# usnistgov/alignn

Measured on AMD Instinct MI355X. Metric: graphs/sec (train fwd+bwd), batch=64 JARVIS-DFT crystals, 4+4 ALIGNN layers, higher is better.
Workload: dtype f32 (projections: split-product MFMA - 3 fp16-slice or 6 bf16-slice products, fp32 accumulate, fp32-grade error)

## Files before the change

alignn_amd/csrc/model.hip:

```cpp
#include <chrono>
#include <cstdio>
#include <cstdlib>
#include <vector>

#include "../../include/alignn_hip.h"
#include "common.h"

namespace {

constexpr int kEvents = 512;
constexpr int kAmaxSlots = 1024;

struct EventPool {
    hipEvent_t ev[kEvents];
    int next = 0;
    bool ok = false;
};
EventPool g_pool[kMaxDevices];

__global__ void fill_kernel(float* __restrict__ p, int64_t n, float v) {
    const int64_t i = (int64_t)blockIdx.x * blockDim.x + threadIdx.x;
    if (i < n) p[i] = v;
}
__global__ void bump_kernel(int64_t* const* __restrict__ ptrs, int n) {
    const int i = blockIdx.x * blockDim.x + threadIdx.x;
    if (i < n) ptrs[i][0] += 1;
}
__global__ __launch_bounds__(256) void transpose_kernel(const float* __restrict__ in, int64_t ld, int rows, int cols,
                                                        float* __restrict__ out) {
    __shared__ float tile[32][33];
    const int tx = threadIdx.x & 31, ty = threadIdx.x >> 5;
    const int r0 = blockIdx.y * 32, c0 = blockIdx.x * 32;
    for (int j = ty; j < 32; j += 8)
        if (r0 + j < rows && c0 + tx < cols) tile[j][tx] = in[(int64_t)(r0 + j) * ld + c0 + tx];
    __syncthreads();
    for (int j = ty; j < 32; j += 8)
        if (c0 + j < cols && r0 + tx < rows) out[(int64_t)(c0 + j) * rows + r0 + tx] = tile[tx][j];
}

struct Act {
    float* p = nullptr;
    float* amax = nullptr;
    float* xn = nullptr;
    float* stat = nullptr;
    float* red = nullptr;
    bool on_T = false;
};
struct Grad {
    float* p = nullptr;
    bool on_T = false;
    bool pre_red = false;
};

struct MlpTape {
    const alignn_mlp_params* p = nullptr;
    Act x, y;
    float *pre = nullptr, *stat = nullptr;
    int64_t rows = 0;
    bool lane = false;
};
struct ConvTape {
    const alignn_conv_params* p = nullptr;
    const alignn_graph_csr* g = nullptr;
    Act x, y, x_out, y_out;
    float *P = nullptr, *M = nullptr, *xpre = nullptr, *s0 = nullptr, *hh = nullptr, *n_stat = nullptr, *e_stat = nullptr;
    bool lane = false, need_y = true;
};
struct Tape {
    float *bl = nullptr, *rbf_e = nullptr, *rbf_a = nullptr, *pool = nullptr;
    float *hcos_buf = nullptr, *pred = nullptr, *seed = nullptr, *g_r = nullptr;
    const float* hcos = nullptr;
    bool angle_fused = false, angle_lane = false;
    float *a_stat1 = nullptr, *a_stat2 = nullptr, *a_scal = nullptr;
    MlpTape atom, e1, e2, a1, a2;
    std::vector<ConvTape> convs;
};

std::vector<std::pair<size_t, size_t>> g_dbg_allocs;
bool dbg_allocs_on() {
    static int on = -1;
    if (on < 0) on = getenv("ALIGNN_AMD_DEBUG_ALLOCS") ? 1 : 0;
    return on == 1;
}

struct Ctx {
    const alignn_model_desc* d;
    const alignn_model_batch* b;
    char* base;
    size_t off = 0, cap = 0;
    bool launch = false;
    bool unsupported = false;
    int unsupported_line = 0;
    int rc = 0;
    hipStream_t main = nullptr, T = nullptr, side = nullptr, aux = nullptr;
    float* amax_arena = nullptr;
    int amax_next = 0;
    EventPool* pool = nullptr;

    float* alloc(size_t floats) {
        const size_t bytes = al256(floats * sizeof(float));
        float* p = reinterpret_cast<float*>(base + off);
        if (launch && dbg_allocs_on()) g_dbg_allocs.emplace_back(off, bytes);
        off += bytes;
        if (launch && off > cap && rc == 0) rc = (int)hipErrorInvalidValue;
        return p;
    }
    size_t sbase[4] = {0, 0, 0, 0}, scur[4] = {0, 0, 0, 0}, speak[4] = {0, 0, 0, 0};
    int which(hipStream_t st) const { return st == main ? 0 : st == T ? 1 : st == side ? 2 : 3; }
    void tmp_reset(hipStream_t st) { scur[which(st)] = 0; }
    float* tmp(hipStream_t st, size_t floats) {
// ... 7 lines not shown
    }
    float* new_amax() {
        if (amax_next >= kAmaxSlots) {
            if (rc == 0) rc = (int)hipErrorInvalidValue;
            return amax_arena;
        }
        return amax_arena + amax_next++;
    }
    float* new_amax2() {
        if (amax_next + 2 > kAmaxSlots) {
            if (rc == 0) rc = (int)hipErrorInvalidValue;
            return amax_arena;
        }
        amax_next += 2;
        return amax_arena + amax_next - 2;
    }
    bool track(int64_t rows) const { return rows >= d->amax_min_rows; }
    const alignn_ff_desc* ff = nullptr;
    bool param_grads = true;
    bool geom = false;
    float *g_rbf_e = nullptr, *g_rbf_a = nullptr;
    bool g_rbf_a_on_T = false;
    ptrdiff_t toff = 0;
    float* sink = nullptr;
    int64_t sink_floats = 0;
    ptrdiff_t sink_toff = 0;
    float* twin(float* dW) const { return dW + ((sink != nullptr && dW >= sink && dW < sink + sink_floats) ? sink_toff : toff); }
    int n_sync = 0, n_launch = 0;
    double t_sync = 0.0;
    bool timing = false;
    void sync(hipStream_t waiter, hipStream_t src) {
        if (!launch || rc != 0 || waiter == src) return;
        const auto t0 = timing ? std::chrono::steady_clock::now() : std::chrono::steady_clock::time_point();
        hipEvent_t e = pool->ev[pool->next];
        pool->next = (pool->next + 1) % kEvents;
        rc = (int)hipEventRecord(e, src);
        if (rc == 0) rc = (int)hipStreamWaitEvent(waiter, e, 0);
        ++n_sync;
        if (timing) t_sync += std::chrono::duration<double>(std::chrono::steady_clock::now() - t0).count();
    }
};

#define UNSUP()                         \
    do {                                \
        c.unsupported = true;           \
        if (!c.unsupported_line) c.unsupported_line = __LINE__; \
    } while (0)

#define L(call)                                                                                        \
    do {                                                                                               \
        if (c.launch && c.rc == 0) {                                                                   \
            c.rc = (call);                                                                             \
            ++c.n_launch;                                                                              \
            if (c.rc != 0 && getenv("ALIGNN_AMD_DEBUG")) fprintf(stderr, "model.hip:%d rc %d: %s\n", __LINE__, c.rc, #call); \
        }                                                                                              \
    } while (0)

inline bool x6_shape_ok(const Ctx& c, int64_t M, int64_t lda, int N, int K) {
    const int64_t tiles = ((M + 63) / 64) * ((N + 255) / 256);
    return tiles >= c.d->x6_min_tiles && (lda % 4) == 0 && alignn_gemm_nt_x6_supported(M, N, K) != 0;
}

void fill(Ctx& c, float* p, int64_t n, float v, hipStream_t st) {
    if (!c.launch || c.rc != 0 || n <= 0) return;
    hipLaunchKernelGGL(fill_kernel, dim3((unsigned)((n + 255) / 256)), dim3(256), 0, st, p, n, v);
    c.rc = (int)hipGetLastError();
}

void project(Ctx& c, const float* a, int64_t lda, const float* a_amax, const float* w, int64_t ldw, const void* img,
             const float* w_amax, const float* bias, float* out, int64_t ldo, int64_t M, int N, int K, hipStream_t st) {
    if (x6_shape_ok(c, M, lda, N, K)) {
        if (a_amax == nullptr || img == nullptr) {
// ... 7 lines not shown
}

void bn_finalize_folded(Ctx& c, float* partial, int slabs, int64_t rows, int F, const float* gamma, const float* beta,
                        float* rm, float* rv, float* stat, hipStream_t st) {
    if (slabs > kFoldAbove) {
        float* fold = c.alloc((size_t)alignn_slab_fold_slabs() * 2 * F);
        L(alignn_slab_fold(partial, slabs, 2 * F, fold, st));
        partial = fold;
        slabs = alignn_slab_fold_slabs();
    }
    L(alignn_bn_finalize(partial, slabs, rows, F, gamma, beta, c.d->eps, c.d->momentum, rm, rv, stat, st));
}

void bn_bwd_finalize_folded(Ctx& c, float* partial, int slabs, int F, float* red, hipStream_t st) {
    if (slabs > kFoldAbove) {
        float* fold = c.alloc((size_t)alignn_slab_fold_slabs() * 2 * F);
        L(alignn_slab_fold(partial, slabs, 2 * F, fold, st));
        partial = fold;
        slabs = alignn_slab_fold_slabs();
    }
    L(alignn_bn_bwd_finalize(partial, slabs, F, red, st));
}



Act mlp_fwd(Ctx& c, MlpTape& t, const alignn_mlp_params& p, const Act& x, int64_t rows) {
    const bool ln = c.d->norm == 1;
    const int F = p.out, K = p.in;
    t.p = &p;
    t.x = x;
    t.rows = rows;
    t.lane = c.T != c.main && rows >= c.d->lane_min_rows;
    hipStream_t st = t.lane ? c.T : c.main;
    if (t.lane != x.on_T) c.sync(st, x.on_T ? c.T : c.main);
    t.pre = c.alloc((size_t)rows * F);
    t.stat = c.alloc(ln ? (size_t)rows * 2 : (size_t)4 * F);
    const bool fused_stats = !ln && x.amax != nullptr && x6_shape_ok(c, rows, K, F, K);
    if (fused_stats) {
        if (p.img == nullptr) {
            UNSUP();
            return Act{};
        }
        const int tiles = alignn_gemm_nt_x6_row_tiles(rows, F, K);
        float* partial = c.alloc((size_t)(tiles + 1) * 2 * F);
        L(alignn_gemm_nt_f16x3_stats(x.p, K, x.amax, p.img, p.w_amax, p.b, t.pre, F, rows, F, K, partial, st));
        bn_finalize_folded(c, partial, tiles, rows, F, p.gamma, p.beta, p.rm, p.rv, t.stat, st);
    } else {
        project(c, x.p, K, x.amax, p.W, K, p.img, p.w_amax, p.b, t.pre, F, rows, F, K, st);
        if (!ln) {
            const int slabs = alignn_col_stats_slabs(rows);
            float* partial = c.alloc((size_t)slabs * (3 * F + 1));
            L(alignn_col_stats_welford(t.pre, F, rows, F, partial, st));
            L(alignn_bn_finalize_welford(partial, slabs, rows, F, p.gamma, p.beta, c.d->eps, c.d->momentum, p.rm, p.rv, t.stat, st));
        }
    }
    Act y;
    y.p = c.alloc((size_t)rows * F);
    y.amax = c.track(rows) ? c.new_amax() : nullptr;
    if (ln)
        L(alignn_ln_silu_fwd(t.pre, F, nullptr, 0, p.gamma, p.beta, c.d->eps, y.p, F, t.stat, rows, F, y.amax, st));
    else {
        L(alignn_bn_silu_fwd(t.pre, F, nullptr, 0, t.stat, y.p, F, rows, F, y.amax, st));
        y.xn = t.pre;
        y.stat = t.stat;
        y.red = p.red;
    }
    y.on_T = t.lane;
    t.y = y;
    return y;
}

void conv_fwd(Ctx& c, ConvTape& t, const alignn_conv_params& p, const alignn_graph_csr& g, const Act& x, const Act& y,
              bool need_y) {
    const bool ln = c.d->norm == 1;
    const int H = c.d->H, Kin = H;
    const int64_t n = g.n, m = g.m;
    t.p = &p;
    t.g = &g;
    t.x = x;
    t.y = y;
    t.need_y = need_y;
    t.lane = c.T != c.main && m >= c.d->lane_min_rows;
    hipStream_t main = c.main, T = t.lane ? c.T : c.main;
    if (x.on_T) c.sync(main, c.T);
    if (!t.lane && y.on_T) c.sync(main, c.T);
    t.P = c.alloc((size_t)n * 4 * H);
    project(c, x.p, Kin, x.amax, p.wcat, Kin, p.wcat_img, p.wcat_amax, p.bcat, t.P, 4 * H, n, 4 * H, Kin, main);
    t.xpre = c.alloc((size_t)n * H);
    t.s0 = c.alloc((size_t)n * H);
    t.hh = c.alloc((size_t)n * H);
    t.M = c.alloc((size_t)m * H);
    const int n_slabs = alignn_egc_slabs(n);
    float *n_part = nullptr, *e_part = nullptr;
    if (ln)
        t.n_stat = c.alloc((size_t)n * 2);
    else {
        n_part = c.alloc((size_t)n_slabs * (3 * H + 1));
        t.n_stat = c.alloc((size_t)8 * H);
        t.e_stat = t.n_stat + 4 * H;
    }
    const bool x6 = x6_shape_ok(c, m, Kin, H, Kin);
    const bool pre_added = y.amax != nullptr && x6;
    if (!pre_added && x6) UNSUP();
    if (t.lane) c.sync(T, main);
    Act yo;
    if (need_y) {
        yo.p = c.alloc((size_t)m * H);
        yo.amax = c.track(m) ? c.new_amax() : nullptr;
        if (ln) t.e_stat = c.alloc((size_t)m * 2);
        yo.on_T = t.lane;
    }
    bool y_normed = false;
    if (pre_added) {
        if (p.weg_img == nullptr) {
            UNSUP();
            return;
        }
        const int tiles = alignn_gemm_nt_x6_row_tiles(m, H, Kin);
        if (!ln) e_part = c.alloc((size_t)(tiles + 1) * 2 * H);
        if (c.d->bd_segment_table && g.seg_node != nullptr && g.seg_rank != nullptr) {
            float* bd2 = c.alloc((size_t)n * H);
            L(alignn_gather_rows_ld(t.P + H, 4 * H, g.seg_node, bd2, H, n, H, T));
            L(alignn_gemm_nt_f16x3_gather2(y.p, Kin, y.amax, p.weg_img, p.weg_amax, p.b_eg, t.M, H, m, H, Kin, t.P, 4 * H, g.src,
                                           bd2, H, g.seg_rank, e_part, T));
        } else
            L(alignn_gemm_nt_f16x3_gather(y.p, Kin, y.amax, p.weg_img, p.weg_amax, p.b_eg, t.M, H, m, H, Kin, t.P, 4 * H, g.src,
                                          g.dst, e_part, T));
        if (!ln) bn_finalize_folded(c, e_part, tiles, m, H, p.e_gamma, p.e_beta, p.e_rm, p.e_rv, t.e_stat, T);
        y_normed = need_y && (!ln || alignn_egc_ln_fused_supported(H, m));
        if (!y_normed)
            L(alignn_egc_gate_fwd_pre(t.P, t.M, g.seg_ptr, g.seg_node, g.src, n, m, H, t.xpre, t.s0, t.hh, nullptr, n_part, T));
        else if (ln)
            L(alignn_egc_gate_fwd_pre_ln(t.P, t.M, g.seg_ptr, g.seg_node, g.src, n, m, H, t.xpre, t.s0, t.hh, p.e_gamma, p.e_beta, c.d->eps,
                                         y.p, yo.p, t.e_stat, yo.amax, T));
        else
            L(alignn_egc_gate_fwd_pre_norm(t.P, t.M, g.seg_ptr, g.seg_node, g.src, n, m, H, t.xpre, t.s0, t.hh, n_part, t.e_stat,
                                           y.p, yo.p, yo.amax, T));
    } else {
        L(alignn_gemm_nt(y.p, Kin, p.w_eg, Kin, p.b_eg, nullptr, 0, t.M, H, m, H, Kin, T));
        if (!ln) e_part = c.alloc((size_t)n_slabs * (3 * H + 1));
        L(alignn_egc_gate_fwd(t.P, t.M, g.seg_ptr, g.seg_node, g.src, n, m, H, t.xpre, t.s0, t.hh, e_part, n_part, T));
    }
    if (t.lane) c.sync(main, T);
// ... 55 lines not shown
    fill(c, c.amax_arena, kAmaxSlots, 0.0f, c.main);
    const bool angle_first = c.ff == nullptr && d.norm == 0 && d.angle_fused != 0 && Tn > 0 && c.T != c.main && Tn >= d.lane_min_rows &&
                             alignn_angle_embed_supported(d.angle_bins, d.angle1.out, d.angle2.out) != 0;
    if (angle_first) c.sync(c.T, c.main);
    const bool prep_aside = angle_first && c.aux != c.main && d.n_weights > 0 && c.ff == nullptr &&
                            !x6_shape_ok(c, N, d.atom.in, d.atom.out, d.atom.in) &&
                            !x6_shape_ok(c, E, d.edge1.in, d.edge1.out, d.edge1.in);
    hipStream_t prep_st = prep_aside ? c.aux : c.main;
    if (prep_aside) c.sync(c.aux, c.main);
    if (d.n_weights > 0) L(alignn_prepare_weights(d.weight_descs, d.n_weights, d.weight_amax, prep_st));
    if (d.n_bump > 0 && c.launch && c.rc == 0) {
        hipLaunchKernelGGL(bump_kernel, dim3((d.n_bump + 63) / 64), dim3(64), 0, c.main, (int64_t* const*)d.bump_ptrs, d.n_bump);
        c.rc = (int)hipGetLastError();
    }
    tp.hcos = b.h;
    if (c.ff != nullptr && c.ff->lg_on_fly) {
        tp.hcos_buf = c.alloc((size_t)Tn);
        L(alignn_bond_cosine_fwd(b.r, b.lg.src, b.lg.dst, tp.hcos_buf, Tn, c.main));
        tp.hcos = tp.hcos_buf;
    }
    if (!angle_first) c.sync(c.T, c.main);
    Act z;
    tp.angle_fused = d.norm == 0 && d.angle_fused != 0 && Tn > 0 &&
                     alignn_angle_embed_supported(d.angle_bins, d.angle1.out, d.angle2.out) != 0;
    if (tp.angle_fused) {
        tp.angle_lane = c.T != c.main && Tn >= d.lane_min_rows;
        hipStream_t st = tp.angle_lane ? c.T : c.main;
        tp.a_stat1 = c.alloc((size_t)4 * d.angle1.out);
        tp.a_stat2 = c.alloc((size_t)4 * d.angle2.out);
        tp.a_scal = c.alloc((size_t)alignn_angle_embed_scal_floats());
        alignn_angle_args a = angle_args(c, tp);
        z.p = c.alloc((size_t)Tn * H);
        z.amax = c.track(Tn) ? c.new_amax() : nullptr;
        z.on_T = tp.angle_lane;
        a.z = z.p;
        a.z_amax = z.amax;
        a.workspace_bytes = alignn_angle_embed_workspace(Tn, d.angle_bins, 0);
        a.workspace = c.alloc(a.workspace_bytes / sizeof(float));
        L(alignn_angle_embed_fwd(&a, st));
    } else {
        tp.rbf_a = c.alloc((size_t)Tn * d.angle_bins);
        L(alignn_rbf_fwd(tp.hcos, d.angle_centers, d.angle_gamma, tp.rbf_a, Tn, d.angle_bins, c.main));
        Act za;
        za.p = tp.rbf_a;
        z = mlp_fwd(c, tp.a2, d.angle2, mlp_fwd(c, tp.a1, d.angle1, za, Tn), Tn);
    }
    Act xa;
    xa.p = const_cast<float*>(b.atom_features);
    Act x = mlp_fwd(c, tp.atom, d.atom, xa, N);
    tp.bl = c.alloc((size_t)E);
    L(alignn_norm3_fwd(b.r, tp.bl, E, c.main));
    tp.rbf_e = c.alloc((size_t)E * d.edge_bins);
    L(alignn_rbf_fwd(tp.bl, d.edge_centers, d.edge_gamma, tp.rbf_e, E, d.edge_bins, c.main));
    Act ye;
    ye.p = tp.rbf_e;
    Act y1 = mlp_fwd(c, tp.e1, d.edge1, ye, E);
    if (prep_aside) c.sync(c.main, c.aux);
    Act y = mlp_fwd(c, tp.e2, d.edge2, y1, E);
    if (c.unsupported) return;
    tp.convs.assign(conv_count(d), ConvTape{});
    int k = 0;
    for (int i = 0; i < d.alignn_layers; ++i) {
        ConvTape& tg = tp.convs[k];
        conv_fwd(c, tg, d.convs[k], b.g, x, y, true);
        ++k;
        ConvTape& tl = tp.convs[k];
        conv_fwd(c, tl, d.convs[k], b.lg, tg.y_out, z, i + 1 < d.alignn_layers);
        ++k;
        x = tg.x_out;
        y = tl.x_out;
        z = tl.y_out;
        if (c.unsupported) return;
    }
    for (int i = 0; i < d.gcn_layers; ++i) {
        ConvTape& tg = tp.convs[k];
        conv_fwd(c, tg, d.convs[k], b.g, x, y, i + 1 < d.gcn_layers);
        ++k;
        x = tg.x_out;
        y = tg.y_out;
        if (c.unsupported) return;
    }
    if (x.on_T) c.sync(c.main, c.T);
    tp.pool = c.alloc((size_t)b.B * H);
    L(alignn_segment_mean_fwd(x.p, b.graph_ptr, tp.pool, b.B, H, c.main));
    L(alignn_gemm_nt(tp.pool, H, d.fc_W, H, d.fc_b, nullptr, 0, out, d.out_features, b.B, d.out_features, H, c.main));
    c.sync(c.main, c.T);
}


void transpose(Ctx& c, const float* w, int64_t ld, int rows, int cols, float* out, hipStream_t st) {
    if (!c.launch || c.rc != 0) return;
    hipLaunchKernelGGL(transpose_kernel, dim3((cols + 31) / 32, (rows + 31) / 32), dim3(256), 0, st, w, ld, rows, cols, out);
    c.rc = (int)hipGetLastError();
}

void dgrad(Ctx& c, const float* g, int64_t ldg, const float* g_amax, const float* w, int Nred, int Kout, const void* img_t,
           const float* w_amax, const float* addend, int64_t ldadd, float* out, int64_t M, hipStream_t st, const Act* src,
           bool* pre_red) {
    if (pre_red) *pre_red = false;
    const bool x6 = x6_shape_ok(c, M, ldg, Kout, Nred);
    if (x6) {
        if (g_amax == nullptr || img_t == nullptr) {
            UNSUP();
            return;
        }
        if (src != nullptr && src->xn != nullptr) {
            const int tiles = alignn_gemm_nt_x6_row_tiles(M, Kout, Nred);
            float* part = c.alloc((size_t)(tiles + 1) * 2 * Kout);
            L(alignn_gemm_nt_f16x3_bnred(g, ldg, g_amax, img_t, w_amax, nullptr, addend, ldadd, out, Kout, M, Kout, Nred, src->xn,
                                         Kout, src->stat, part, st));
            bn_bwd_finalize_folded(c, part, tiles, Kout, src->red, st);
            if (pre_red) *pre_red = true;
            return;
        }
        L(alignn_gemm_nt_f16x3(g, ldg, g_amax, img_t, w_amax, nullptr, addend, ldadd, out, Kout, M, Kout, Nred, st));
// ... 34 lines not shown

hipStream_t side_for(Ctx& c, int64_t rows) { return (c.side != c.main && rows >= c.d->side_min_rows) ? c.side : c.main; }

float* edge_grad_buffer(Ctx& c, const ConvTape& t, int64_t m, int Kin) {
    if (c.d->reuse_tape && c.ff == nullptr && t.M != nullptr && Kin == c.d->H) return t.M;
    return c.alloc((size_t)m * Kin);
}

bool dgrad_wgrad(Ctx& c, const ConvTape& t, const float* GM, const float* gm_amax, const float* gy, float* g_y, int64_t m, int H,
                 int Kin, hipStream_t st, const Act* src, bool* pre_red) {
    const alignn_conv_params& p = *t.p;
    if (c.d->dw_fused <= 0 || m < c.d->dw_fused || !c.param_grads || gm_amax == nullptr || t.y.amax == nullptr || p.weg_img_t == nullptr || Kin != H ||
        !alignn_gemm_dgrad_wgrad_supported(m, H, Kin) || !x6_shape_ok(c, m, H, Kin, H))
        return false;
    const size_t nb = alignn_gemm_dgrad_wgrad_workspace(m);
    c.tmp_reset(st);
    float* ws = c.tmp(st, nb / 4);
    const int slabs = 2 * alignn_gemm_dgrad_wgrad_slabs(m);
    float* part = src != nullptr ? c.alloc((size_t)slabs * 2 * Kin) : nullptr;
    L(alignn_gemm_dgrad_wgrad_f16x3(GM, H, gm_amax, t.y.p, Kin, t.y.amax, p.weg_img_t, p.weg_amax, gy, H, g_y, Kin,
                                    src != nullptr ? src->xn : nullptr, Kin, src != nullptr ? src->stat : nullptr, part, p.g_weg, Kin, m,
                                    ws, nb, st));
    if (src != nullptr) bn_bwd_finalize_folded(c, part, slabs, Kin, src->red, st);
    if (pre_red) *pre_red = src != nullptr;
    return true;
}

Grad mlp_bwd(Ctx& c, const MlpTape& t, const Grad& gy, bool need_gx) {
    const bool ln = c.d->norm == 1;
    const alignn_mlp_params& p = *t.p;
    const int F = p.out, K = p.in;
    const int64_t rows = t.rows;
    hipStream_t st = t.lane ? c.T : c.main;
    if (t.lane != gy.on_T) c.sync(st, gy.on_T ? c.T : c.main);
    float* gpre = c.alloc((size_t)rows * F);
    float* g_amax = c.track(rows) ? c.new_amax() : nullptr;
    const int slabs = ln ? alignn_ln_slabs(rows) : alignn_col_stats_slabs(rows);
    float* gb_part = nullptr;
    if (ln) {
        float* part = c.alloc((size_t)slabs * 2 * F);
        L(alignn_ln_silu_bwd(gy.p, F, t.pre, F, p.gamma, p.beta, t.stat, gpre, F, part, rows, F, g_amax, st));
        if (c.param_grads) L(alignn_bn_bwd_finalize(part, slabs, F, p.red, st));
    } else {
        if (!gy.pre_red) {
            float* part = c.alloc((size_t)slabs * 2 * F);
            L(alignn_bn_silu_bwd_reduce(gy.p, F, t.pre, F, t.stat, rows, F, part, st));
            L(alignn_bn_bwd_finalize(part, slabs, F, p.red, st));
        }
        if (F <= 1024) {
            gb_part = c.alloc((size_t)slabs * F);
            L(alignn_bn_silu_bwd_apply_sum(gy.p, F, t.pre, F, t.stat, p.red, 0, gpre, F, rows, F, g_amax, gb_part, st));
        } else
            L(alignn_bn_silu_bwd_apply(gy.p, F, t.pre, F, t.stat, p.gamma, p.red, 0, gpre, F, rows, F, g_amax, st));
    }
    Grad gx;
    if (need_gx) {
        gx.p = c.alloc((size_t)rows * K);
        gx.on_T = t.lane;
        const Act* src = (t.x.xn != nullptr && g_amax != nullptr) ? &t.x : nullptr;
        dgrad(c, gpre, F, g_amax, p.W, F, K, p.img_t, p.w_amax, nullptr, 0, gx.p, rows, st, src, &gx.pre_red);
    }
    if (!c.param_grads) return gx;
    hipStream_t sd = side_for(c, rows);
    if (sd != st) {
        c.sync(sd, c.main);
        if (t.lane) c.sync(sd, c.T);
    }
    c.tmp_reset(sd);
    gemm_tn(c, gpre, F, g_amax, t.x.p, K, t.x.amax, p.gW, rows, F, K, sd);
    if (gb_part != nullptr)
        L(alignn_slab_sum(gb_part, slabs, F, p.gb, sd));
    else
        col_sum(c, gpre, F, rows, F, p.gb, sd);
    return gx;
}

void conv_bwd(Ctx& c, const ConvTape& t, const Grad& gx_out, const Grad* gy_out, Grad& g_x, Grad& g_y, bool need_gx = true) {
    const bool ln = c.d->norm == 1;
    const alignn_conv_params& p = *t.p;
    const alignn_graph_csr& g = *t.g;
    const int H = c.d->H, Kin = H;
    const int64_t n = g.n, m = g.m;
    hipStream_t main = c.main, T = t.lane ? c.T : c.main;
    if (gx_out.on_T) c.sync(main, c.T);
    if (!t.lane && gy_out != nullptr && gy_out->on_T) c.sync(main, c.T);
    float* GP = c.alloc((size_t)n * 4 * H);
    float* gp_amax = c.track(n) ? c.new_amax() : nullptr;
    float* gm_amax = c.track(m) ? c.new_amax() : nullptr;
    float* g_xpre = GP + 3 * (size_t)H;
    const int n_slabs = ln ? alignn_ln_slabs(n) : alignn_col_stats_slabs(n);
    float* n_part = c.alloc((size_t)n_slabs * 2 * H);
    float* gs1 = c.alloc((size_t)n * H);
    float* gs0 = c.alloc((size_t)n * H);
    if (ln) {
        L(alignn_ln_silu_bwd_node(gx_out.p, H, t.xpre, H, p.n_gamma, p.n_beta, t.n_stat, g_xpre, 4 * H, n_part, n, H, gp_amax, t.s0, t.hh,
                                  gs1, gs0, main));
        if (c.param_grads) L(alignn_bn_bwd_finalize(n_part, n_slabs, H, p.n_red, main));
    } else {
        L(alignn_bn_silu_bwd_reduce(gx_out.p, H, t.xpre, H, t.n_stat, n, H, n_part, main));
        L(alignn_bn_bwd_finalize(n_part, n_slabs, H, p.n_red, main));
        L(alignn_bn_silu_bwd_apply_node(gx_out.p, H, t.xpre, H, t.n_stat, p.n_gamma, p.n_red, 0, g_xpre, 4 * H, n, H, gp_amax, t.s0,
                                        t.hh, gs1, gs0, main));
    }
    const float* gy = gy_out != nullptr ? gy_out->p : nullptr;
    if (t.lane && gy_out != nullptr && !gy_out->on_T) c.sync(T, main);
    const bool lg_blocks = g.grp_seg_ptr != nullptr;
    const bool dense = lg_blocks && g.dense_max_src > 0 && alignn_egc_bwd_lg_dense_supported(g.dense_max_src);
    const bool ln_inside = ln && gy != nullptr && dense && alignn_egc_ln_fused_supported(H, m);
    const bool ln_dst = ln && gy != nullptr && !lg_blocks && alignn_egc_ln_dst_supported(H);
    const float *ge = gy, *e_stat = t.e_stat, *e_red = nullptr;
    if (ln) {
        ge = e_stat = nullptr;
        if (gy != nullptr && !ln_inside && !ln_dst) {
            float* g_branch = c.alloc((size_t)m * H);
            const int e_slabs = alignn_ln_slabs(m);
            float* e_part = c.alloc((size_t)e_slabs * 2 * H);
            L(alignn_ln_silu_bwd(gy, H, t.M, H, p.e_gamma, p.e_beta, t.e_stat, g_branch, H, e_part, m, H, nullptr, T));
            if (c.param_grads) L(alignn_bn_bwd_finalize(e_part, e_slabs, H, p.e_red, T));
            ge = g_branch;
        }
    } else if (gy != nullptr) {
        if (!gy_out->pre_red) {
            const int e_slabs = alignn_col_stats_slabs(m);
            float* e_part = c.alloc((size_t)e_slabs * 2 * H);
            L(alignn_bn_silu_bwd_reduce(gy, H, t.M, H, t.e_stat, m, H, e_part, T));
            L(alignn_bn_bwd_finalize(e_part, e_slabs, H, p.e_red, T));
        }
        e_red = p.e_red;
    }
    if (t.lane) c.sync(T, main);
    float* GM = c.alloc((size_t)m * H);
    const int gslabs = lg_blocks ? (int)g.n_groups : (ln_dst ? alignn_egc_ln_dst_slabs(n) : alignn_egc_slabs(n));
    float* gb_part = c.alloc((size_t)gslabs * H);
    float* e_part = (ln_inside || ln_dst) ? c.alloc((size_t)gslabs * 2 * H) : nullptr;
    if (ln_inside)
        L(alignn_egc_bwd_lg_dense_ln(gy, t.M, t.P, gs1, gs0, p.e_gamma, p.e_beta, t.e_stat, m, g.grp_seg_ptr, g.grp_src_ptr, g.n_groups,
                                     g.dense_max_src, g.seg_ptr, g.seg_node, H, GM, GP, gb_part, e_part, gm_amax, gp_amax, T));
    else if (dense)
        L(alignn_egc_bwd_lg_dense(ge, t.M, t.P, gs1, gs0, e_stat, e_red, 0, m, g.grp_seg_ptr, g.grp_src_ptr, g.n_groups,
                                  g.dense_max_src, g.seg_ptr, g.seg_node, H, GM, GP, gb_part, gm_amax, gp_amax, T));
    else if (lg_blocks)
        L(alignn_egc_bwd_lg_fused(ge, t.M, t.P, gs1, gs0, e_stat, e_red, 0, m, g.grp_seg_ptr, g.grp_src_ptr, g.n_groups,
                                  g.seg_ptr, g.seg_node, g.dst, g.out_ptr, g.out_slot, H, GM, GP, gb_part, gm_amax, gp_amax, T));
    else if (ln_dst)
        L(alignn_egc_bwd_dst_ln(gy, t.M, t.P, gs1, gs0, p.e_gamma, p.e_beta, t.e_stat, g.seg_ptr, g.seg_node, g.src, n, H, GM, GP, gb_part,
                                e_part, gm_amax, gp_amax, T));
    else
        L(alignn_egc_bwd_dst(ge, t.M, t.P, gs1, gs0, e_stat, p.e_gamma, e_red, 0, m, g.seg_ptr, g.seg_node, g.src, n, H, GM, GP,
                             gb_part, gm_amax, gp_amax, T));
    if (e_part != nullptr && c.param_grads) L(alignn_bn_bwd_finalize(e_part, gslabs, H, p.e_red, T));
    if (!lg_blocks) L(alignn_egc_bwd_src(GM, t.M, gs1, g.out_ptr, g.out_slot, g.dst, n, H, GP, gp_amax, T));
    if (t.lane) c.sync(main, T);
    g_y.p = edge_grad_buffer(c, t, m, Kin);
    hipStream_t sx = main;
    if (need_gx) {
        g_x.p = c.alloc((size_t)n * Kin);
        if (!t.lane && c.aux != main) {
            c.sync(c.aux, main);
            sx = c.aux;
        }
        dgrad(c, GP, 4 * H, gp_amax, p.wcat, 4 * H, Kin, p.wcat_img_t, p.wcat_amax, gx_out.p, H, g_x.p, n, sx, nullptr, nullptr);
    }
    const Act* src = (t.y.xn != nullptr && gm_amax != nullptr) ? &t.y : nullptr;
    const bool dw = dgrad_wgrad(c, t, GM, gm_amax, gy, g_y.p, m, H, Kin, T, src, &g_y.pre_red);
    if (!dw) dgrad(c, GM, H, gm_amax, p.w_eg, H, Kin, p.weg_img_t, p.weg_amax, gy, H, g_y.p, m, T, src, &g_y.pre_red);
    g_y.on_T = t.lane;
    g_x.on_T = false;
    if (sx != main) c.sync(main, sx);
    if (!c.param_grads) return;
    hipStream_t sd = side_for(c, m);
    if (sd != main) {
        c.sync(sd, main);
        if (t.lane) c.sync(sd, c.T);
    } else if (t.lane)
        c.sync(main, c.T);
    c.tmp_reset(sd);
    L(alignn_slab_sum(gb_part, gslabs, H, p.g_beg, sd));
    if (!dw) gemm_tn(c, GM, H, gm_amax, t.y.p, Kin, t.y.amax, p.g_weg, m, H, Kin, sd);
    gemm_tn(c, GP, 4 * H, gp_amax, t.x.p, Kin, t.x.amax, p.g_wcat, n, 4 * H, Kin, sd);
    col_sum(c, GP, 4 * H, n, 4 * H, p.g_bcat, sd);
}

void run_backward(Ctx& c, const Tape& tp, const float* g_out) {
    const alignn_model_desc& d = *c.d;
    const alignn_model_batch& b = *c.b;
    const int64_t N = b.g.n;
    const int H = d.H, OF = d.out_features, B = b.B;
    c.amax_arena = c.alloc(kAmaxSlots);
    c.amax_next = 0;
    fill(c, c.amax_arena, kAmaxSlots, 0.0f, c.main);
    c.sync(c.T, c.main);
    c.sync(c.side, c.main);
    float* g_pool = c.alloc((size_t)B * H);
    dgrad(c, g_out, OF, nullptr, d.fc_W, OF, H, nullptr, nullptr, nullptr, 0, g_pool, B, c.main, nullptr, nullptr);
    if (c.param_grads) {
        c.tmp_reset(c.main);
        gemm_tn(c, g_out, OF, nullptr, tp.pool, H, nullptr, d.g_fc_W, B, OF, H, c.main);
        if ((OF % 4) == 0)
            col_sum(c, g_out, OF, B, OF, d.g_fc_b, c.main);
        else {
            float* ones = c.alloc((size_t)B);
            fill(c, ones, B, 1.0f, c.main);
            gemm_tn(c, g_out, OF, nullptr, ones, 1, nullptr, d.g_fc_b, B, OF, 1, c.main);
        }
    }
    Grad gx;
    gx.p = c.alloc((size_t)N * H);
    L(alignn_segment_mean_bwd(g_pool, b.graph_ptr, gx.p, B, H, c.main));
    int k = conv_count(d) - 1;
    Grad gy, gz;
    bool have_gy = false, have_gz = false;
    for (int i = d.gcn_layers - 1; i >= 0; --i, --k) {
        Grad nx, ny;
        conv_bwd(c, tp.convs[k], gx, have_gy ? &gy : nullptr, nx, ny);
        gx = nx;
        gy = ny;
        have_gy = true;
        if (c.unsupported) return;
    }
    const bool angle_geom = c.geom && c.ff != nullptr && c.ff->lg_on_fly;
    for (int i = d.alignn_layers - 1; i >= 0; --i) {
        Grad gm, nz;
        conv_bwd(c, tp.convs[k], gy, have_gz ? &gz : nullptr, gm, nz);
        --k;
        gz = nz;
        have_gz = true;
        if (i == 0) {
            if (tp.angle_fused) {
                hipStream_t st = tp.angle_lane ? c.T : c.main;
                if (tp.angle_lane != gz.on_T) c.sync(st, gz.on_T ? c.T : c.main);
                alignn_angle_args a = angle_args(c, tp);
                a.gz = gz.p;
                a.workspace_bytes = alignn_angle_embed_workspace(a.rows, d.angle_bins, 1);
                a.workspace = c.alloc(a.workspace_bytes / sizeof(float));
                L(alignn_angle_embed_bwd(&a, st));
            } else if (c.param_grads || angle_geom) {
                Grad ga = mlp_bwd(c, tp.a2, gz, true);
                Grad gr = mlp_bwd(c, tp.a1, ga, angle_geom);
                c.g_rbf_a = gr.p;
                c.g_rbf_a_on_T = gr.on_T;
            }
        }
        Grad nx, ny;
        conv_bwd(c, tp.convs[k], gx, &gm, nx, ny, i > 0 || c.param_grads);
        --k;
        gx = nx;
        gy = ny;
        if (c.unsupported) return;
    }
    if (c.param_grads) mlp_bwd(c, tp.atom, gx, false);
    Grad ge = mlp_bwd(c, tp.e2, gy, true);
    Grad gre = mlp_bwd(c, tp.e1, ge, c.geom);
    c.g_rbf_e = gre.p;
    c.sync(c.main, c.T);
    c.sync(c.main, c.side);
}

Act mlp_infer(Ctx& c, const alignn_mlp_params& p, const Act& x, int64_t rows) {
    const int F = p.out, K = p.in;
    const bool lane = c.T != c.main && rows >= c.d->lane_min_rows;
    hipStream_t st = lane ? c.T : c.main;
    if (lane != x.on_T) c.sync(st, x.on_T ? c.T : c.main);
    float* pre = c.alloc((size_t)rows * F);
    float* stat = c.alloc((size_t)4 * F);
    project(c, x.p, K, x.amax, p.W, K, p.img, p.w_amax, p.b, pre, F, rows, F, K, st);
    L(alignn_bn_finalize(nullptr, 0, rows, F, p.gamma, p.beta, c.d->eps, c.d->momentum, p.rm, p.rv, stat, st));
    Act y;
    y.p = c.alloc((size_t)rows * F);
    y.amax = c.track(rows) ? c.new_amax() : nullptr;
    L(alignn_bn_silu_fwd(pre, F, nullptr, 0, stat, y.p, F, rows, F, y.amax, st));
    y.on_T = lane;
    return y;
}

void conv_infer(Ctx& c, const alignn_conv_params& p, const alignn_graph_csr& g, const Act& x, const Act& y, bool need_y,
                Act& x_out, Act& y_out) {
    const int H = c.d->H, Kin = H;
    const int64_t n = g.n, m = g.m;
    const bool lane = c.T != c.main && m >= c.d->lane_min_rows;
    hipStream_t main = c.main, T = lane ? c.T : c.main;
    if (x.on_T) c.sync(main, c.T);
    if (!lane && y.on_T) c.sync(main, c.T);
    float* P = c.alloc((size_t)n * 4 * H);
    project(c, x.p, Kin, x.amax, p.wcat, Kin, p.wcat_img, p.wcat_amax, p.bcat, P, 4 * H, n, 4 * H, Kin, main);
    float* stats = c.alloc((size_t)8 * H);
    L(alignn_bn_finalize(nullptr, 0, n, H, p.n_gamma, p.n_beta, c.d->eps, c.d->momentum, p.n_rm, p.n_rv, stats, main));
    L(alignn_bn_finalize(nullptr, 0, m, H, p.e_gamma, p.e_beta, c.d->eps, c.d->momentum, p.e_rm, p.e_rv, stats + 4 * H, main));
    if (lane) c.sync(T, main);
    float* Cm = c.alloc((size_t)m * H);
    project(c, y.p, Kin, y.amax, p.w_eg, Kin, p.weg_img, p.weg_amax, p.b_eg, Cm, H, m, H, Kin, T);
    float* xpre = c.alloc((size_t)n * H);
    Act yo;
    if (need_y) {
        yo.p = c.alloc((size_t)m * H);
        yo.amax = c.track(m) ? c.new_amax() : nullptr;
        yo.on_T = lane;
    }
    L(alignn_egc_gate_infer(P, Cm, g.seg_ptr, g.seg_node, g.src, n, m, H, xpre, stats + 4 * H, y.p, yo.p, yo.amax, T));
    if (lane) c.sync(main, T);
    x_out = Act{};
    x_out.p = c.alloc((size_t)n * H);
    x_out.amax = c.track(n) ? c.new_amax() : nullptr;
    L(alignn_bn_silu_fwd(xpre, H, x.p, Kin, stats, x_out.p, H, n, H, x_out.amax, main));
    y_out = yo;
}

void run_infer(Ctx& c, float* out) {
    const alignn_model_desc& d = *c.d;
    const alignn_model_batch& b = *c.b;
    const int64_t N = b.g.n, E = b.g.m, Tn = b.lg.m;
    c.amax_arena = c.alloc(kAmaxSlots);
    c.amax_next = 0;
    fill(c, c.amax_arena, kAmaxSlots, 0.0f, c.main);
    if (d.n_weights > 0) L(alignn_prepare_weights(d.weight_descs, d.n_weights, d.weight_amax, c.main));
    c.sync(c.T, c.main);
    Act z;
    if (d.angle_fused != 0 && Tn > 0 && alignn_angle_embed_supported(d.angle_bins, d.angle1.out, d.angle2.out) != 0) {
        const bool lane = c.T != c.main && Tn >= d.lane_min_rows;
        Tape tp;
        tp.hcos = b.h;
        tp.a_stat1 = c.alloc((size_t)4 * d.angle1.out);
        tp.a_stat2 = c.alloc((size_t)4 * d.angle2.out);
        tp.a_scal = c.alloc((size_t)alignn_angle_embed_scal_floats());
        alignn_angle_args a = angle_args(c, tp);
        z.p = c.alloc((size_t)Tn * d.H);
        z.amax = c.track(Tn) ? c.new_amax() : nullptr;
        z.on_T = lane;
        a.z = z.p;
        a.z_amax = z.amax;
        L(alignn_angle_embed_infer(&a, lane ? c.T : c.main));
    } else {
        float* rbf_a = c.alloc((size_t)Tn * d.angle_bins);
        L(alignn_rbf_fwd(b.h, d.angle_centers, d.angle_gamma, rbf_a, Tn, d.angle_bins, c.main));
        Act za;
        za.p = rbf_a;
        z = mlp_infer(c, d.angle2, mlp_infer(c, d.angle1, za, Tn), Tn);
    }
    Act xa;
    xa.p = const_cast<float*>(b.atom_features);
    Act x = mlp_infer(c, d.atom, xa, N);
    float* bl = c.alloc((size_t)E);
    L(alignn_norm3_fwd(b.r, bl, E, c.main));
    float* rbf_e = c.alloc((size_t)E * d.edge_bins);
    L(alignn_rbf_fwd(bl, d.edge_centers, d.edge_gamma, rbf_e, E, d.edge_bins, c.main));
    Act ye;
    ye.p = rbf_e;
    Act y = mlp_infer(c, d.edge2, mlp_infer(c, d.edge1, ye, E), E);
    if (c.unsupported) return;
    int k = 0;
    for (int i = 0; i < d.alignn_layers; ++i) {
        Act xo, m_, yo, zo;
        conv_infer(c, d.convs[k++], b.g, x, y, true, xo, m_);
        conv_infer(c, d.convs[k++], b.lg, m_, z, i + 1 < d.alignn_layers, yo, zo);
        x = xo, y = yo, z = zo;
        if (c.unsupported) return;
    }
    for (int i = 0; i < d.gcn_layers; ++i) {
        Act xo, yo;
        conv_infer(c, d.convs[k++], b.g, x, y, i + 1 < d.gcn_layers, xo, yo);
        x = xo, y = yo;
        if (c.unsupported) return;
    }
    if (x.on_T) c.sync(c.main, c.T);
    float* pool = c.alloc((size_t)b.B * d.H);
    L(alignn_segment_mean_fwd(x.p, b.graph_ptr, pool, b.B, d.H, c.main));
    L(alignn_gemm_nt(pool, d.H, d.fc_W, d.H, d.fc_b, nullptr, 0, out, d.out_features, b.B, d.out_features, d.H, c.main));
    c.sync(c.main, c.T);
}


void run_ff_eval(Ctx& c, Tape& tp, float* out, float* forces, float* stress) {
    const alignn_model_desc& d = *c.d;
    const alignn_model_batch& b = *c.b;
    const alignn_ff_desc& f = *c.ff;
    const int64_t N = b.g.n, E = b.g.m, Tn = b.lg.m;
    const int B = b.B;
    c.param_grads = false;
    c.geom = true;
    tp.pred = c.alloc((size_t)B);
    tp.seed = c.alloc((size_t)B);
    run_forward(c, tp, tp.pred);
    if (c.unsupported) return;
    L(alignn_ff_energy(tp.pred, tp.bl, b.graph_ptr, B, E, f.energy_mult_natoms, f.use_penalty, f.penalty_factor, f.penalty_threshold,
                       out, tp.seed, c.main));
    run_backward(c, tp, tp.seed);
    if (c.unsupported) return;
    float* g_bl = c.alloc((size_t)E);
    L(alignn_rbf_bwd(tp.bl, d.edge_centers, d.edge_gamma, c.g_rbf_e, g_bl, E, d.edge_bins, c.main));
    if (f.use_penalty) L(alignn_ff_penalty_bwd(tp.bl, g_bl, E, B, f.penalty_factor, f.penalty_threshold, c.main));
    float* gr_bl = c.alloc((size_t)3 * E);
    L(alignn_norm3_bwd(b.r, g_bl, gr_bl, E, c.main));
    tp.g_r = gr_bl;
    if (f.lg_on_fly) {
        float* g_h = c.alloc((size_t)Tn);
        L(alignn_rbf_bwd(tp.hcos, d.angle_centers, d.angle_gamma, c.g_rbf_a, g_h, Tn, d.angle_bins, c.main));
        float* ga = c.alloc((size_t)3 * Tn);
// ... 442 lines not shown
}

int open_ctx(Ctx& c, const Plan* pl, size_t workspace_bytes, alignn_stream_t stream, bool need_full) {
    c.cap = workspace_bytes;
    set_streams(c, stream);
    if (pl == nullptr)
        c.side = c.aux = c.main;
    else {
        if (pl->unsupported) return (int)hipErrorNotSupported;
        const bool full = workspace_bytes >= pl->total();
        if (!full && (need_full || workspace_bytes < pl->fwd_total())) return (int)hipErrorInvalidValue;
        pl->place_scratch(c, full);
    }
    if ((c.T != c.main || c.side != c.main || c.aux != c.main) && !take_pool(c)) return (int)hipErrorNotInitialized;
    return 0;
}

}

extern "C" {

size_t alignn_ff_desc_sizeof(void) { return sizeof(alignn_ff_desc); }

int alignn_debug_allocs(size_t* out, int cap) {
    const int n = (int)g_dbg_allocs.size();
    for (int i = 0; i < n && i < cap; ++i) {
        out[2 * i] = g_dbg_allocs[i].first;
        out[2 * i + 1] = g_dbg_allocs[i].second;
    }
    g_dbg_allocs.clear();
    return n;
}

int alignn_ff_plan(const alignn_model_desc* d, const alignn_model_batch* b, const alignn_ff_desc* f, size_t* eval_bytes,
                   size_t* total_bytes) {
    if (!ff_ok(d, b, f) || eval_bytes == nullptr || total_bytes == nullptr) return (int)hipErrorInvalidValue;
    Plan pl = make_plan(d, b, f, nullptr);
    if (pl.unsupported) {
        if (getenv("ALIGNN_AMD_DEBUG")) fprintf(stderr, "alignn_ff_plan: kernel choice not carried (model.hip:%d)\n", pl.line);
        return (int)hipErrorNotSupported;
    }
    *eval_bytes = pl.fwd_total();
    *total_bytes = pl.total();
    return pl.rc;
}

int alignn_ff_eval(const alignn_model_desc* d, const alignn_model_batch* b, const alignn_ff_desc* f, void* workspace,
                   size_t workspace_bytes, float* out, float* forces, float* stress, alignn_stream_t stream) {
    if (!ff_ok(d, b, f) || workspace == nullptr || out == nullptr || forces == nullptr) return (int)hipErrorInvalidValue;
    const Plan pl = make_plan(d, b, f, stream);
    Ctx c{d, b, static_cast<char*>(workspace)};
    c.ff = f;
    if (const int rc = open_ctx(c, &pl, workspace_bytes, stream, false)) return rc;
    c.launch = true;
    Tape tp;
    run_ff_eval(c, tp, out, forces, stress);
    if (c.unsupported) return (int)hipErrorNotSupported;
    return c.rc;
}

int alignn_ff_grad(const alignn_model_desc* d, const alignn_model_batch* b, const alignn_ff_desc* f, void* workspace,
                   size_t workspace_bytes, const float* g_out, const float* g_forces, const float* g_stress, float* gflat,
                   float* gflat_t, int64_t grad_floats, float* gsink, float* gsink_t, int64_t sink_floats, alignn_stream_t stream) {
    if (!ff_ok(d, b, f) || workspace == nullptr || gflat == nullptr || gflat_t == nullptr || grad_floats <= 0 || (grad_floats & 3))
        return (int)hipErrorInvalidValue;
    if (gsink != nullptr && (gsink_t == nullptr || sink_floats <= 0 || (sink_floats & 3) || !aligned16(gsink) ||
// ... 129 lines not shown
```

Measured before the change: 4438.

## Track per-tensor readiness events and overlap node-branch backward across streams

Replaces the boolean on_T flag with a Ready record holding the producing stream and an optional event, so consumers wait on the exact event instead of a fresh full-stream sync. The node-gradient part of each conv backward is split into conv_bwd_node and, in ALIGNN layers, issued for the graph conv before the line-graph conv, possibly on the aux stream. The node dgrad's result is no longer joined back to main immediately but marked and joined lazily. This aims to overlap independent backward work and remove serialising syncs, at the cost of more event bookkeeping, a risk of event pool wraparound (guarded by an error), and extra atomic debug counters.

New measurement: 4492 (median of 6 runs). +1.2%, better.

```diff
diff --git a/alignn_amd/csrc/model.hip b/alignn_amd/csrc/model.hip
--- a/alignn_amd/csrc/model.hip
+++ b/alignn_amd/csrc/model.hip
@@ -1,3 +1,4 @@
+#include <atomic>
 #include <chrono>
 #include <cstdio>
 #include <cstdlib>
@@ -38,17 +39,22 @@
         if (c0 + j < cols && r0 + tx < rows) out[(int64_t)(c0 + j) * rows + r0 + tx] = tile[tx][j];
 }
 
+struct Ready {
+    hipStream_t st = nullptr;
+    hipEvent_t ev = nullptr;
+    int at = 0;
+};
 struct Act {
     float* p = nullptr;
     float* amax = nullptr;
     float* xn = nullptr;
     float* stat = nullptr;
     float* red = nullptr;
-    bool on_T = false;
+    Ready rdy;
 };
 struct Grad {
     float* p = nullptr;
-    bool on_T = false;
+    Ready rdy;
     bool pre_red = false;
 };
 
@@ -76,6 +82,7 @@
     std::vector<ConvTape> convs;
 };
 
+std::atomic<int64_t> g_dbg_aux_marks{0}, g_dbg_late_waits{0}, g_dbg_max_dist{0};
 std::vector<std::pair<size_t, size_t>> g_dbg_allocs;
 bool dbg_allocs_on() {
     static int on = -1;
@@ -149,12 +156,63 @@
     void sync(hipStream_t waiter, hipStream_t src) {
         if (!launch || rc != 0 || waiter == src) return;
         const auto t0 = timing ? std::chrono::steady_clock::now() : std::chrono::steady_clock::time_point();
+        wait(waiter, mark(src));
+        ++n_sync;
+        if (timing) t_sync += std::chrono::duration<double>(std::chrono::steady_clock::now() - t0).count();
+    }
+    int n_mark = 0;
+    hipEvent_t mark(hipStream_t src) {
+        if (!launch || rc != 0) return nullptr;
         hipEvent_t e = pool->ev[pool->next];
         pool->next = (pool->next + 1) % kEvents;
         rc = (int)hipEventRecord(e, src);
-        if (rc == 0) rc = (int)hipStreamWaitEvent(waiter, e, 0);
-        ++n_sync;
-        if (timing) t_sync += std::chrono::duration<double>(std::chrono::steady_clock::now() - t0).count();
+        ++n_mark;
+        return e;
+    }
+    void wait(hipStream_t waiter, hipEvent_t e) {
+        if (!launch || rc != 0 || e == nullptr) return;
+        rc = (int)hipStreamWaitEvent(waiter, e, 0);
+    }
+    hipStream_t where(const Ready& r) const { return r.st != nullptr ? r.st : main; }
+    Ready by(hipStream_t st) const {
+        Ready r;
+        r.st = st;
+        return r;
+    }
+    Ready marked(hipStream_t st) {
+        Ready r = by(st);
+        if (st != main) {
+            r.ev = mark(st);
+            r.at = n_mark;
+            if (st == aux && r.ev != nullptr) {
+                aux_at = r.at;
+                g_dbg_aux_marks.fetch_add(1, std::memory_order_relaxed);
+            }
+        }
+        return r;
+    }
+    void need(hipStream_t reader, const Ready& r) {
+        const hipStream_t src = where(r);
+        if (src == reader) return;
+        if (r.ev == nullptr) {
+            sync(reader, src);
+            return;
+        }
+        if (!launch || rc != 0) return;
+        const int dist = n_mark - r.at;
+        g_dbg_late_waits.fetch_add(1, std::memory_order_relaxed);
+        if (dist > g_dbg_max_dist.load(std::memory_order_relaxed)) g_dbg_max_dist.store(dist, std::memory_order_relaxed);
+        if (dist >= kEvents - 1) {
+            rc = (int)hipErrorInvalidValue;
+            return;
+        }
+        wait(reader, r.ev);
+        if (reader == main && src == aux && r.at == aux_at) aux_at = 0;
+    }
+    int aux_at = 0;
+    void join_aux() {
+        if (aux_at != 0) sync(main, aux);
+        aux_at = 0;
     }
 };
 
@@ -228,7 +286,7 @@
     t.rows = rows;
     t.lane = c.T != c.main && rows >= c.d->lane_min_rows;
     hipStream_t st = t.lane ? c.T : c.main;
-    if (t.lane != x.on_T) c.sync(st, x.on_T ? c.T : c.main);
+    c.need(st, x.rdy);
     t.pre = c.alloc((size_t)rows * F);
     t.stat = c.alloc(ln ? (size_t)rows * 2 : (size_t)4 * F);
     const bool fused_stats = !ln && x.amax != nullptr && x6_shape_ok(c, rows, K, F, K);
@@ -261,7 +319,7 @@
         y.stat = t.stat;
         y.red = p.red;
     }
-    y.on_T = t.lane;
+    y.rdy = c.by(st);
     t.y = y;
     return y;
 }
@@ -278,8 +336,8 @@
     t.need_y = need_y;
     t.lane = c.T != c.main && m >= c.d->lane_min_rows;
     hipStream_t main = c.main, T = t.lane ? c.T : c.main;
-    if (x.on_T) c.sync(main, c.T);
-    if (!t.lane && y.on_T) c.sync(main, c.T);
+    c.need(main, x.rdy);
+    if (!t.lane) c.need(main, y.rdy);
     t.P = c.alloc((size_t)n * 4 * H);
     project(c, x.p, Kin, x.amax, p.wcat, Kin, p.wcat_img, p.wcat_amax, p.bcat, t.P, 4 * H, n, 4 * H, Kin, main);
     t.xpre = c.alloc((size_t)n * H);
@@ -304,7 +362,7 @@
         yo.p = c.alloc((size_t)m * H);
         yo.amax = c.track(m) ? c.new_amax() : nullptr;
         if (ln) t.e_stat = c.alloc((size_t)m * 2);
-        yo.on_T = t.lane;
+        yo.rdy = c.by(T);
     }
     bool y_normed = false;
     if (pre_added) {
@@ -426,7 +484,7 @@
         alignn_angle_args a = angle_args(c, tp);
         z.p = c.alloc((size_t)Tn * H);
         z.amax = c.track(Tn) ? c.new_amax() : nullptr;
-        z.on_T = tp.angle_lane;
+        z.rdy = c.by(st);
         a.z = z.p;
         a.z_amax = z.amax;
         a.workspace_bytes = alignn_angle_embed_workspace(Tn, d.angle_bins, 0);
@@ -474,7 +532,7 @@
         y = tg.y_out;
         if (c.unsupported) return;
     }
-    if (x.on_T) c.sync(c.main, c.T);
+    c.need(c.main, x.rdy);
     tp.pool = c.alloc((size_t)b.B * H);
     L(alignn_segment_mean_fwd(x.p, b.graph_ptr, tp.pool, b.B, H, c.main));
     L(alignn_gemm_nt(tp.pool, H, d.fc_W, H, d.fc_b, nullptr, 0, out, d.out_features, b.B, d.out_features, H, c.main));
@@ -575,7 +633,7 @@
     const int F = p.out, K = p.in;
     const int64_t rows = t.rows;
     hipStream_t st = t.lane ? c.T : c.main;
-    if (t.lane != gy.on_T) c.sync(st, gy.on_T ? c.T : c.main);
+    c.need(st, gy.rdy);
     float* gpre = c.alloc((size_t)rows * F);
     float* g_amax = c.track(rows) ? c.new_amax() : nullptr;
     const int slabs = ln ? alignn_ln_slabs(rows) : alignn_col_stats_slabs(rows);
@@ -599,7 +657,7 @@
     Grad gx;
     if (need_gx) {
         gx.p = c.alloc((size_t)rows * K);
-        gx.on_T = t.lane;
+        gx.rdy = c.by(st);
         const Act* src = (t.x.xn != nullptr && g_amax != nullptr) ? &t.x : nullptr;
         dgrad(c, gpre, F, g_amax, p.W, F, K, p.img_t, p.w_amax, nullptr, 0, gx.p, rows, st, src, &gx.pre_red);
     }
@@ -618,35 +676,52 @@
     return gx;
 }
 
-void conv_bwd(Ctx& c, const ConvTape& t, const Grad& gx_out, const Grad* gy_out, Grad& g_x, Grad& g_y, bool need_gx = true) {
+struct NodeBranch {
+    float *GP = nullptr, *gp_amax = nullptr, *gm_amax = nullptr, *gs1 = nullptr, *gs0 = nullptr;
+    Ready rdy;
+};
+NodeBranch conv_bwd_node(Ctx& c, const ConvTape& t, const Grad& gx_out) {
+    const bool ln = c.d->norm == 1;
+    const alignn_conv_params& p = *t.p;
+    const int H = c.d->H;
+    const int64_t n = t.g->n, m = t.g->m;
+    hipStream_t st = (!t.lane && c.aux != c.main && c.where(gx_out.rdy) == c.aux) ? c.aux : c.main;
+    c.need(st, gx_out.rdy);
+    NodeBranch nb;
+    nb.GP = c.alloc((size_t)n * 4 * H);
+    nb.gp_amax = c.track(n) ? c.new_amax() : nullptr;
+    nb.gm_amax = c.track(m) ? c.new_amax() : nullptr;
+    float* g_xpre = nb.GP + 3 * (size_t)H;
+    const int n_slabs = ln ? alignn_ln_slabs(n) : alignn_col_stats_slabs(n);
+    float* n_part = c.alloc((size_t)n_slabs * 2 * H);
+    nb.gs1 = c.alloc((size_t)n * H);
+    nb.gs0 = c.alloc((size_t)n * H);
+    if (ln) {
+        L(alignn_ln_silu_bwd_node(gx_out.p, H, t.xpre, H, p.n_gamma, p.n_beta, t.n_stat, g_xpre, 4 * H, n_part, n, H, nb.gp_amax, t.s0,
+                                  t.hh, nb.gs1, nb.gs0, st));
+        if (c.param_grads) L(alignn_bn_bwd_finalize(n_part, n_slabs, H, p.n_red, st));
+    } else {
+        L(alignn_bn_silu_bwd_reduce(gx_out.p, H, t.xpre, H, t.n_stat, n, H, n_part, st));
+        L(alignn_bn_bwd_finalize(n_part, n_slabs, H, p.n_red, st));
+        L(alignn_bn_silu_bwd_apply_node(gx_out.p, H, t.xpre, H, t.n_stat, p.n_gamma, p.n_red, 0, g_xpre, 4 * H, n, H, nb.gp_amax, t.s0,
+                                        t.hh, nb.gs1, nb.gs0, st));
+    }
+    nb.rdy = c.marked(st);
+    return nb;
+}
+
+void conv_bwd(Ctx& c, const ConvTape& t, const NodeBranch& nb, const Grad& gx_out, const Grad* gy_out, Grad& g_x, Grad& g_y,
+              bool need_gx = true) {
     const bool ln = c.d->norm == 1;
     const alignn_conv_params& p = *t.p;
     const alignn_graph_csr& g = *t.g;
     const int H = c.d->H, Kin = H;
     const int64_t n = g.n, m = g.m;
     hipStream_t main = c.main, T = t.lane ? c.T : c.main;
-    if (gx_out.on_T) c.sync(main, c.T);
-    if (!t.lane && gy_out != nullptr && gy_out->on_T) c.sync(main, c.T);
-    float* GP = c.alloc((size_t)n * 4 * H);
-    float* gp_amax = c.track(n) ? c.new_amax() : nullptr;
-    float* gm_amax = c.track(m) ? c.new_amax() : nullptr;
-    float* g_xpre = GP + 3 * (size_t)H;
-    const int n_slabs = ln ? alignn_ln_slabs(n) : alignn_col_stats_slabs(n);
-    float* n_part = c.alloc((size_t)n_slabs * 2 * H);
-    float* gs1 = c.alloc((size_t)n * H);
-    float* gs0 = c.alloc((size_t)n * H);
-    if (ln) {
-        L(alignn_ln_silu_bwd_node(gx_out.p, H, t.xpre, H, p.n_gamma, p.n_beta, t.n_stat, g_xpre, 4 * H, n_part, n, H, gp_amax, t.s0, t.hh,
-                                  gs1, gs0, main));
-        if (c.param_grads) L(alignn_bn_bwd_finalize(n_part, n_slabs, H, p.n_red, main));
-    } else {
-        L(alignn_bn_silu_bwd_reduce(gx_out.p, H, t.xpre, H, t.n_stat, n, H, n_part, main));
-        L(alignn_bn_bwd_finalize(n_part, n_slabs, H, p.n_red, main));
-        L(alignn_bn_silu_bwd_apply_node(gx_out.p, H, t.xpre, H, t.n_stat, p.n_gamma, p.n_red, 0, g_xpre, 4 * H, n, H, gp_amax, t.s0,
-                                        t.hh, gs1, gs0, main));
-    }
+    float *GP = nb.GP, *gp_amax = nb.gp_amax, *gm_amax = nb.gm_amax, *gs1 = nb.gs1, *gs0 = nb.gs0;
+    if (!t.lane && gy_out != nullptr) c.need(main, gy_out->rdy);
     const float* gy = gy_out != nullptr ? gy_out->p : nullptr;
-    if (t.lane && gy_out != nullptr && !gy_out->on_T) c.sync(T, main);
+    if (t.lane && gy_out != nullptr) c.need(T, gy_out->rdy);
     const bool lg_blocks = g.grp_seg_ptr != nullptr;
     const bool dense = lg_blocks && g.dense_max_src > 0 && alignn_egc_bwd_lg_dense_supported(g.dense_max_src);
     const bool ln_inside = ln && gy != nullptr && dense && alignn_egc_ln_fused_supported(H, m);
@@ -671,6 +746,7 @@
         }
         e_red = p.e_red;
     }
+    c.need(main, nb.rdy);
     if (t.lane) c.sync(T, main);
     float* GM = c.alloc((size_t)m * H);
     const int gslabs = lg_blocks ? (int)g.n_groups : (ln_dst ? alignn_egc_ln_dst_slabs(n) : alignn_egc_slabs(n));
@@ -702,14 +778,14 @@
             c.sync(c.aux, main);
             sx = c.aux;
         }
+        c.need(sx, gx_out.rdy);
         dgrad(c, GP, 4 * H, gp_amax, p.wcat, 4 * H, Kin, p.wcat_img_t, p.wcat_amax, gx_out.p, H, g_x.p, n, sx, nullptr, nullptr);
     }
     const Act* src = (t.y.xn != nullptr && gm_amax != nullptr) ? &t.y : nullptr;
     const bool dw = dgrad_wgrad(c, t, GM, gm_amax, gy, g_y.p, m, H, Kin, T, src, &g_y.pre_red);
     if (!dw) dgrad(c, GM, H, gm_amax, p.w_eg, H, Kin, p.weg_img_t, p.weg_amax, gy, H, g_y.p, m, T, src, &g_y.pre_red);
-    g_y.on_T = t.lane;
-    g_x.on_T = false;
-    if (sx != main) c.sync(main, sx);
+    g_y.rdy = c.by(T);
+    if (need_gx) g_x.rdy = c.marked(sx);
     if (!c.param_grads) return;
     hipStream_t sd = side_for(c, m);
     if (sd != main) {
@@ -755,7 +831,8 @@
     bool have_gy = false, have_gz = false;
     for (int i = d.gcn_layers - 1; i >= 0; --i, --k) {
         Grad nx, ny;
-        conv_bwd(c, tp.convs[k], gx, have_gy ? &gy : nullptr, nx, ny);
+        const NodeBranch nb = conv_bwd_node(c, tp.convs[k], gx);
+        conv_bwd(c, tp.convs[k], nb, gx, have_gy ? &gy : nullptr, nx, ny);
         gx = nx;
         gy = ny;
         have_gy = true;
@@ -763,15 +840,17 @@
     }
     const bool angle_geom = c.geom && c.ff != nullptr && c.ff->lg_on_fly;
     for (int i = d.alignn_layers - 1; i >= 0; --i) {
+        const NodeBranch nb_g = conv_bwd_node(c, tp.convs[k - 1], gx);
         Grad gm, nz;
-        conv_bwd(c, tp.convs[k], gy, have_gz ? &gz : nullptr, gm, nz);
+        const NodeBranch nb_lg = conv_bwd_node(c, tp.convs[k], gy);
+        conv_bwd(c, tp.convs[k], nb_lg, gy, have_gz ? &gz : nullptr, gm, nz);
         --k;
         gz = nz;
         have_gz = true;
         if (i == 0) {
             if (tp.angle_fused) {
                 hipStream_t st = tp.angle_lane ? c.T : c.main;
-                if (tp.angle_lane != gz.on_T) c.sync(st, gz.on_T ? c.T : c.main);
+                c.need(st, gz.rdy);
                 alignn_angle_args a = angle_args(c, tp);
                 a.gz = gz.p;
                 a.workspace_bytes = alignn_angle_embed_workspace(a.rows, d.angle_bins, 1);
@@ -781,11 +860,11 @@
                 Grad ga = mlp_bwd(c, tp.a2, gz, true);
                 Grad gr = mlp_bwd(c, tp.a1, ga, angle_geom);
                 c.g_rbf_a = gr.p;
-                c.g_rbf_a_on_T = gr.on_T;
+                c.g_rbf_a_on_T = c.where(gr.rdy) != c.main;
             }
         }
         Grad nx, ny;
-        conv_bwd(c, tp.convs[k], gx, &gm, nx, ny, i > 0 || c.param_grads);
+        conv_bwd(c, tp.convs[k], nb_g, gx, &gm, nx, ny, i > 0 || c.param_grads);
         --k;
         gx = nx;
         gy = ny;
@@ -795,6 +874,7 @@
     Grad ge = mlp_bwd(c, tp.e2, gy, true);
     Grad gre = mlp_bwd(c, tp.e1, ge, c.geom);
     c.g_rbf_e = gre.p;
+    c.join_aux();
     c.sync(c.main, c.T);
     c.sync(c.main, c.side);
 }
@@ -803,7 +883,7 @@
     const int F = p.out, K = p.in;
     const bool lane = c.T != c.main && rows >= c.d->lane_min_rows;
     hipStream_t st = lane ? c.T : c.main;
-    if (lane != x.on_T) c.sync(st, x.on_T ? c.T : c.main);
+    c.need(st, x.rdy);
     float* pre = c.alloc((size_t)rows * F);
     float* stat = c.alloc((size_t)4 * F);
     project(c, x.p, K, x.amax, p.W, K, p.img, p.w_amax, p.b, pre, F, rows, F, K, st);
@@ -812,7 +892,7 @@
     y.p = c.alloc((size_t)rows * F);
     y.amax = c.track(rows) ? c.new_amax() : nullptr;
     L(alignn_bn_silu_fwd(pre, F, nullptr, 0, stat, y.p, F, rows, F, y.amax, st));
-    y.on_T = lane;
+    y.rdy = c.by(st);
     return y;
 }
 
@@ -822,8 +902,8 @@
     const int64_t n = g.n, m = g.m;
     const bool lane = c.T != c.main && m >= c.d->lane_min_rows;
     hipStream_t main = c.main, T = lane ? c.T : c.main;
-    if (x.on_T) c.sync(main, c.T);
-    if (!lane && y.on_T) c.sync(main, c.T);
+    c.need(main, x.rdy);
+    if (!lane) c.need(main, y.rdy);
     float* P = c.alloc((size_t)n * 4 * H);
     project(c, x.p, Kin, x.amax, p.wcat, Kin, p.wcat_img, p.wcat_amax, p.bcat, P, 4 * H, n, 4 * H, Kin, main);
     float* stats = c.alloc((size_t)8 * H);
@@ -837,7 +917,7 @@
     if (need_y) {
         yo.p = c.alloc((size_t)m * H);
         yo.amax = c.track(m) ? c.new_amax() : nullptr;
-        yo.on_T = lane;
+        yo.rdy = c.by(T);
     }
     L(alignn_egc_gate_infer(P, Cm, g.seg_ptr, g.seg_node, g.src, n, m, H, xpre, stats + 4 * H, y.p, yo.p, yo.amax, T));
     if (lane) c.sync(main, T);
@@ -868,7 +948,7 @@
         alignn_angle_args a = angle_args(c, tp);
         z.p = c.alloc((size_t)Tn * d.H);
         z.amax = c.track(Tn) ? c.new_amax() : nullptr;
-        z.on_T = lane;
+        z.rdy = c.by(lane ? c.T : c.main);
         a.z = z.p;
         a.z_amax = z.amax;
         L(alignn_angle_embed_infer(&a, lane ? c.T : c.main));
@@ -904,7 +984,7 @@
         x = xo, y = yo;
         if (c.unsupported) return;
     }
-    if (x.on_T) c.sync(c.main, c.T);
+    c.need(c.main, x.rdy);
     float* pool = c.alloc((size_t)b.B * d.H);
     L(alignn_segment_mean_fwd(x.p, b.graph_ptr, pool, b.B, d.H, c.main));
     L(alignn_gemm_nt(pool, d.H, d.fc_W, d.H, d.fc_b, nullptr, 0, out, d.out_features, b.B, d.out_features, d.H, c.main));
@@ -1413,6 +1493,13 @@
     return n;
 }
 
+int alignn_debug_joins(int64_t* out) {
+    out[0] = g_dbg_aux_marks.exchange(0);
+    out[1] = g_dbg_late_waits.exchange(0);
+    out[2] = g_dbg_max_dist.exchange(0);
+    return 0;
+}
+
 int alignn_ff_plan(const alignn_model_desc* d, const alignn_model_batch* b, const alignn_ff_desc* f, size_t* eval_bytes,
                    size_t* total_bytes) {
     if (!ff_ok(d, b, f) || eval_bytes == nullptr || total_bytes == nullptr) return (int)hipErrorInvalidValue;
```
